# willwng/madrona_rl_envs_playground

Hardware: AMD Instinct MI355X
Metric: env-steps/sec (whole node), Overcooked 32768 worlds, random policy (higher is better)
Workload: dtype u8; 1 GPU; Overcooked cramped_room, 32768 worlds per GPU, horizon 400, uniform random actions (pre-sampled pool of 64, resident in HBM); worlds_per_gpu=32768, obs_gather=False

## Files before the change

### madrona_rl_envs_playground_amd/csrc/capi.hip

```cpp
#include "common.hpp"
#include "episode_scan.hpp"

#include <algorithm>
#include <cstring>
#include <exception>
#include <map>
#include <mutex>
#include <string>

namespace mrl {

static thread_local char g_error[512] = "";

static const char *const kDebugKeys[] = {
    "overcooked.wpw",
    "overcooked.whole_max",
    "overcooked.lds_max",
    "overcooked.share_max_players",
    "overcooked.share_private",
    "overcooked.no_share",
    "overcooked.lds_pad",
    "overcooked.no_fixed",
    "overcooked.no_direct",
    "overcooked.whole_store",
    "overcooked.store_policy",
    "overcooked.wide_rollout",
    "overcooked.groups",
    "overcooked.shared_consts",
    "overcooked.variant",
    "hanabi.variant",
    "hanabi.pairing",
    "hanabi.no_persistent",
    "cartpole.no_persistent",
    "cartpole.persistent_max",
    "cartpole.variant",
    "fused_step",
    "fused_heal_test",
    "inject_scan_timeout",
    "ablate",
    "stamps",
};
static std::mutex g_debug_mutex;
static std::map<std::string, int64_t> g_debug;

int64_t debug_get(const char *key, int64_t fallback)
{
    std::lock_guard<std::mutex> lock(g_debug_mutex);
    auto it = g_debug.find(key);
    return it == g_debug.end() ? fallback : it->second;
}

void set_error(const char *fmt, ...)
{
    va_list ap;
    va_start(ap, fmt);
    vsnprintf(g_error, sizeof(g_error), fmt, ap);
    va_end(ap);
}

void bind_device(int gpu_id)
{
    int count = 0;
// ... 484 lines not shown
```

### madrona_rl_envs_playground_amd/csrc/overcooked.hip

```cpp
#include "common.hpp"
#include "random_policy.hpp"
#include "world_reset.hpp"

#include <algorithm>
#include <cstdlib>
#include <cstring>

namespace {

constexpr int kWave = 64;
#ifndef MRL_OVERCOOKED_WPB
#define MRL_OVERCOOKED_WPB 4
#endif
constexpr int kWavesPerBlock = MRL_OVERCOOKED_WPB;
constexpr int kBlock = kWave * kWavesPerBlock;
constexpr int kRowsPerPass = 128;

enum : uint32_t { A_NORTH = 0, A_SOUTH = 1, A_EAST = 2, A_WEST = 3, A_STAY = 4, A_INTERACT = 5 };
enum : uint32_t { T_AIR = 0, T_POT, T_COUNTER, T_ONION_SRC, T_TOMATO_SRC, T_DISH_SRC, T_SERVING };
enum : uint32_t { O_NONE = 0, O_TOMATO, O_ONION, O_DISH, O_SOUP };
constexpr uint32_t kItemNone = 0xFF000000u;
constexpr uint32_t kMaxIngredients = 3;

constexpr uint32_t kConstTerrain = 0;
// ... 23 lines not shown
#endif
    uint32_t whole;
    uint32_t share;
    uint32_t team;
    uint32_t steady;
    uint32_t tail_even;
    uint32_t private_consts;
    uint32_t starts_w;
    uint32_t off_terr;
    uint32_t store_policy;
    uint32_t patch;
    uint32_t unaligned;
    const uint16_t *terr_off;
    uint32_t terr_entries;
    uint32_t direct;
    const uint32_t *hold_tab;
    uint32_t hold_entries;
    uint32_t off_pl, off_x, off_sum, off_cur, off_flags, off_list, off_tail, off_tile;
    uint32_t lds_wave_stride;
    int64_t horizon;
    const uint32_t *consts;
    uint32_t *cell_obj;
    uint2 *players;
    int32_t *timestep;
    const int32_t *actions;
    const long long *actions64;
    int32_t *action_mirror;
    int32_t *reward;
    int32_t *done;
    uint8_t *obs;
    uint64_t ring_stride;
    uint32_t ring_slots, ring_first;
    uint32_t pair_exchange;
};

__device__ __forceinline__ void wave_lds_sync()
{
    __builtin_amdgcn_wave_barrier();
    asm volatile("" ::: "memory");
}

__device__ __forceinline__ uint32_t lds_addr(const void *p)
{
    return (uint32_t)reinterpret_cast<uintptr_t>(p);
}

__device__ __forceinline__ void lds_store_tail_a4(uint8_t *ptr, const uint4 &t)
{
    asm volatile("ds_write_b32 %0, %1\n\t"
                 "ds_write_b32 %0, %2 offset:4\n\t"
                 "ds_write_b32 %0, %3 offset:8\n\t"
                 "ds_write_b32 %0, %4 offset:12"
                 :
                 : "v"(lds_addr(ptr)), "v"(t.x), "v"(t.y), "v"(t.z), "v"(t.w)
                 : "memory");
}

__device__ __forceinline__ void lds_store_tail_a2(uint8_t *ptr, const uint4 &t)
{
    const uint32_t m1 = __builtin_amdgcn_alignbit(t.y, t.x, 16);
    const uint32_t m2 = __builtin_amdgcn_alignbit(t.z, t.y, 16);
    const uint32_t m3 = __builtin_amdgcn_alignbit(t.w, t.z, 16);
    asm volatile("ds_write_b16 %0, %1\n\t"
                 "ds_write_b32 %0, %2 offset:2\n\t"
                 "ds_write_b32 %0, %3 offset:6\n\t"
                 "ds_write_b32 %0, %4 offset:10\n\t"
// ... 135 lines not shown
    const int32_t tick = (int8_t)(o >> 24);
    const uint32_t hname = h & 0xFF;
    const bool is_soup = oname == O_SOUP, in_pot = terr == T_POT;
    const bool idle = is_soup & in_pot & (tick < 0);
    const bool hot = is_soup & in_pot & (tick >= 0);
    const bool plated = is_soup & !in_pot;
    const bool hsoup = hname == O_SOUP;
    const uint32_t idle_on = idle ? on : 0u, idle_tom = idle ? tom : 0u;
    const uint32_t soup_on = hsoup ? (h >> 8) & 0xFF : ((hot | plated) ? on : 0u);
    const uint32_t soup_tom = hsoup ? (h >> 16) & 0xFF : ((hot | plated) ? tom : 0u);
    const uint32_t remaining = (hot & !hsoup) ? (uint32_t)(need - tick) & 0xFF : 0u;
    const uint32_t ready = (hsoup | plated | (hot & (tick >= need))) ? 1u : 0u;
    const uint32_t dish = ((oname == O_DISH) | (hname == O_DISH)) ? 1u : 0u;
    const uint32_t onion = ((oname == O_ONION) | (hname == O_ONION)) ? 1u : 0u;
    const uint32_t tomato = ((oname == O_TOMATO) | (hname == O_TOMATO)) ? 1u : 0u;
    const uint32_t tbit = terr == T_AIR ? 0u : 1u;
    const uint32_t tsh = ((terr - 1u) & 3u) * 8u;
    uint4 t;
    t.x = (terr >= 1 && terr <= 4) ? (tbit << tsh) : 0u;
    t.y = ((terr >= 5) ? (tbit << tsh) : 0u) | (idle_on << 16) | (idle_tom << 24);
    t.z = soup_on | (soup_tom << 8) | (remaining << 16) | (ready << 24);
    t.w = dish | (onion << 8) | (tomato << 16) | ((urgent ? 1u : 0u) << 24);
    return t;
}

__device__ __forceinline__ uint32_t swap_pair(uint32_t v)
{
    return (uint32_t)__builtin_amdgcn_mov_dpp((int)v, 0xB1, 0xF, 0xF, true);
}

template <int kP>
__device__ __forceinline__ void transition_lanes(const StepParams &p, const uint8_t *s_terrain, uint32_t *obj_w, uint32_t *s_x,
                                                 uint32_t *s_sum, uint32_t *s_blk, uint32_t P, uint32_t lane, bool active, uint32_t wl,
                                                 uint32_t q, uint32_t a, uint32_t &posori, uint32_t &held, int32_t &reward_world)
{
    const uint32_t pos = posori & 0xFFu, ori = (posori >> 8) & 0xFFu;
    const uint32_t tgt = pos + (uint32_t)step_of(ori, p.deltas);
    const uint32_t terr = s_terrain[tgt];
    const uint32_t ahead = s_terrain[pos + (uint32_t)step_of(a, p.deltas)];
    const bool inter = active && a == A_INTERACT;
    const bool touches = inter && (terr == T_COUNTER || terr == T_POT);
    const uint32_t key = touches ? tgt : 0xFFFFu;
    const uint32_t base = wl * P;
    uint32_t rank = 0;
    if constexpr (kP == 2) {
        const uint32_t other = swap_pair(key);
        rank = (q == 1u && touches && other == tgt) ? 1u : 0u;
    } else {
        s_x[lane] = key;
        wave_lds_sync();
        for (uint32_t q2 = 0; q2 + 1 < P; q2++) rank += (q2 < q && touches && s_x[base + q2] == key) ? 1u : 0u;
        wave_lds_sync();
    }
    int32_t mine = 0;
    const int32_t value = (int32_t)lookup16(p.values_w, recipe_of(held));
    uint32_t *cell = obj_w + (touches ? tgt : 0u);
    constexpr uint32_t kRounds = kP == 2 ? 2u : 4u;
#pragma clang loop unroll(disable)
    for (uint32_t r = 0; r < kRounds; r++) {
        const bool todo = inter && rank == r;
        if (r > 0 && __ballot(todo) == 0ull) break;
        if (todo) {
            uint32_t there = touches ? *cell : kItemNone;
            const int32_t need = (int32_t)lookup16(p.times_w, recipe_of(there));
            held = interact(p, need, value, terr, held, there, mine);
            if (touches) *cell = there;
        }
        wave_lds_sync();
    }
    uint32_t prop = pos, pori = ori;
    {
        const bool moves = a != A_INTERACT;
        const uint32_t np = pos + (uint32_t)step_of(a, p.deltas);
        pori = (moves && a != A_STAY) ? a : ori;
        prop = (moves && ahead == T_AIR) ? np : pos;
    }
    bool blocked;
    if constexpr (kP == 2) {
        reward_world = mine + (int32_t)swap_pair((uint32_t)mine);
        const uint32_t o = swap_pair(pos | (prop << 8));
        const uint32_t opos = o & 0xFFu, oprop = o >> 8;
        blocked = (prop == oprop) | ((prop == opos) & (pos == oprop));
    } else {
        s_x[lane] = pos | (prop << 8);
        if (active && q == 0) {
            s_sum[wl] = 0u;
            s_blk[wl] = 0u;
        }
        wave_lds_sync();
        if (mine != 0) atomicAdd(&s_sum[wl], (uint32_t)mine);
        bool hit = false;
        for (uint32_t q2 = 0; q2 < P; q2++) {
            const uint32_t v = s_x[base + q2];
            hit |= (q2 != q) & ((prop == (v >> 8)) | ((prop == (v & 0xFFu)) & (pos == (v >> 8))));
        }
        if (hit && active) s_blk[wl] = 1u;
        wave_lds_sync();
        reward_world = active ? (int32_t)s_sum[wl] : 0;
        blocked = active && s_blk[wl] != 0u;
        wave_lds_sync();
    }
    posori = (blocked ? pos : prop) | (pori << 8);
}

__device__ __forceinline__ void tick_pots_world(const StepParams &p, const uint8_t *s_pots, uint32_t *obj, bool valid)
{
    if (valid) {
        for (uint32_t k = 0; k < p.num_pots; k++) {
            const uint32_t c = k < 4 ? (p.pots_w >> (8 * k)) & 0xFFu : (uint32_t)s_pots[k];
            const uint32_t o = obj[c];
            const int32_t tick = (int8_t)(o >> 24);
            if ((o & 0xFF) == O_SOUP && tick >= 0 && tick < (int32_t)lookup16(p.times_w, recipe_of(o)))
                obj[c] = (o & 0x00FFFFFFu) | ((uint32_t)(uint8_t)(tick + 1) << 24);
        }
    }
}
__device__ __forceinline__ void tick_pots(const StepParams &p, const uint8_t *s_pots, uint32_t *s_obj, uint32_t nw, uint32_t lane)
{
    tick_pots_world(p, s_pots, s_obj + lane * p.C, lane < nw);
}
template <bool kPlain = false>
__device__ __forceinline__ void stream_store_rsrc(__amdgpu_buffer_rsrc_t rsrc, uint32_t byte_offset, const uint4 &v)
{
    u32x4 r;
    r.x = v.x;
    r.y = v.y;
    r.z = v.z;
    r.w = v.w;
#ifndef MRL_WHOLE_STORE_AUX
#define MRL_WHOLE_STORE_AUX 16
#endif
    __builtin_amdgcn_raw_buffer_store_b128(r, rsrc, (int)byte_offset, 0, kPlain ? 0 : MRL_WHOLE_STORE_AUX);
}

template <bool kPlain = false>
__device__ __forceinline__ void observe_whole(const StepParams &p, const uint8_t *s_terrain, const uint32_t *s_obj,
                                              const uint32_t *s_pl, const uint8_t *s_cur, const uint8_t *s_flags,
                                              uint8_t *s_tile, uint32_t P, uint32_t w0, uint32_t nw, uint32_t lane,
                                              bool prezeroed = false)
{
    const uint32_t C = p.C, F = p.F, shift = 5 * P, ncells = nw * C;
#ifdef MRL_DIAG
    if (p.ablate & 8u) return;
#endif
    uint8_t *gobs = p.obs + (size_t)w0 * p.block_bytes;
    const uint32_t nbytes = min(nw, w0 < p.num_worlds ? p.num_worlds - w0 : 0u) * p.block_bytes;
    const uint32_t mis = (uint32_t)(reinterpret_cast<uintptr_t>(gobs) & 15u);
    uint8_t *tile = s_tile + mis;
    if (!prezeroed) {
        const uint32_t nchunks = (mis + nbytes + 15u) >> 4;
        for (uint32_t k = lane; k < nchunks; k += kWave) reinterpret_cast<uint4 *>(s_tile)[k] = make_uint4(0, 0, 0, 0);
    }
    wave_lds_sync();
    const uint32_t plane = __umul24(C, F);
    for (uint32_t i = lane; i < ncells; i += kWave) {
        const uint32_t l = __umulhi(i, p.inv_c), c = i - __umul24(l, C);
        const uint32_t terr = s_terrain[c];
        const uint32_t o = s_obj[i];
        const uint32_t who = s_cur[i];
        const uint32_t urgent = s_flags[l];
        const bool occupied = who != 0xFF;
        const uint32_t pidx = (__umul24(l, P) + (occupied ? who : 0u)) * 2;
        const uint32_t w_ori = (s_pl[pidx] >> 8) & 0xFF;
        const uint32_t h = occupied ? s_pl[pidx + 1] : kItemNone;
        const uint4 t = cell_tail(p, terr, o, h, urgent);
// ... 49 lines not shown
        for (int k = 0; k < kBatch; k++) {
            if (i0 + (uint32_t)k * kWave >= ncells) break;
            const uint32_t i = i0 + (uint32_t)k * kWave + lane;
            const bool dyn = i < ncells && (((o[k] & 0xFFu) != O_NONE) | (who[k] != 0xFFu));
            const unsigned long long m = __ballot(dyn);
            const uint32_t before = __builtin_amdgcn_mbcnt_hi((uint32_t)(m >> 32), __builtin_amdgcn_mbcnt_lo((uint32_t)m, 0u));
            if (dyn) s_list[ndyn + before] = (uint16_t)i;
            ndyn += (uint32_t)__popcll(m);
        }
    }
    wave_lds_sync();
    return ndyn;
}

constexpr int kHoldPerLane = 4;
struct HoldTab {
    uint32_t e[kHoldPerLane];
};
__device__ __forceinline__ void hold_request(const StepParams &p, uint32_t lane, HoldTab &h)
{
    const __amdgpu_buffer_rsrc_t tab = __builtin_amdgcn_make_buffer_rsrc(const_cast<uint32_t *>(p.hold_tab), 0, (int)(p.hold_entries * 4u), 0x00020000);
#pragma unroll
    for (int k = 0; k < kHoldPerLane; k++) {
        if ((uint32_t)k * kWave >= p.hold_entries) {
            h.e[k] = 0;
            continue;
        }
        h.e[k] = (uint32_t)__builtin_amdgcn_raw_buffer_load_b32(tab, (int)((lane + (uint32_t)k * kWave) * 4u), 0, 0);
    }
}
template <int kP, bool kUndo>
__device__ __forceinline__ void patch_direct(const StepParams &p, uint32_t *s_obj, const uint8_t *s_flags, const HoldTab &hold,
                                             uint8_t *tile, uint32_t P, uint32_t nw, bool active, uint32_t wl, uint32_t q, uint32_t posori,
                                             uint32_t held)
{
    const uint32_t C = p.C, F = p.F, shift = 5 * P, ncells = nw * C;
    const uint32_t plane = __umul24(C, F);
    const uint32_t ori = (posori >> 8) & 0xFFu;
#pragma unroll
    for (int k = 0; k < kHoldPerLane; k++) {
        if (k > 0 && (uint32_t)k * kWave >= p.hold_entries) break;
        const uint32_t e = hold.e[k];
        const uint32_t i = (e >> 16) & 0x3FFFu;
        const bool holder = ((e >> 30) & 1u) != 0u && i < ncells;
        uint32_t o = s_obj[holder ? i : 0u];
        if (!kUndo && holder && (e >> 31)) {
            const int32_t tick = (int8_t)(o >> 24);
            if ((o & 0xFFu) == O_SOUP && tick >= 0 && tick < (int32_t)lookup16(p.times_w, recipe_of(o))) {
                o = (o & 0x00FFFFFFu) | ((uint32_t)(uint8_t)(tick + 1) << 24);
                s_obj[i] = o;
            }
        }
        const bool player = k == 0 && active;
        if (player || (holder && (o & 0xFFu) != O_NONE)) {
            const uint32_t l = player ? wl : __umulhi(i, p.inv_c);
            const uint32_t terr = player ? (uint32_t)T_AIR : ((e >> 31) ? (uint32_t)T_POT : (uint32_t)T_COUNTER);
            const uint4 t = cell_tail(p, terr, (player || kUndo) ? (uint32_t)kItemNone : o, (player && !kUndo) ? held : (uint32_t)kItemNone, s_flags[l]);
            uint8_t *row0 = tile + (player ? __umul24(l, p.block_bytes) + __umul24(posori & 0xFFu, F) : (e & 0xFFFFu));
            auto viewer_row = [&](uint32_t v, uint8_t *row) {
                lds_store_tail_even(row + shift, t);
                if (player) {
                    const uint32_t rel = q == v ? 0u : (q < v ? q + 1u : q);
                    row[rel] = kUndo ? 0 : 1;
                    row[P + 4 * rel + ori] = kUndo ? 0 : 1;
                }
            };
            if constexpr (kP == 2) {
                viewer_row(0, row0);
                viewer_row(1, row0 + plane);
            } else {
                for (uint32_t v = 0; v < P; v++) viewer_row(v, row0 + __umul24(v, plane));
            }
        }
    }
}

template <int kP, bool kRestore, bool kPlain = false>
__device__ __forceinline__ void observe_patch(const StepParams &p, const uint8_t *s_terrain, uint32_t *s_obj,
                                              const uint32_t *s_pl, const uint8_t *s_cur, const uint8_t *s_flags, uint8_t *s_prev,
                                              const uint16_t *s_list, uint32_t ndyn, uint8_t *tile, uint32_t P, uint32_t w0, uint32_t l0,
                                              uint32_t nl, uint32_t lane, const HoldTab &hold, bool active, uint32_t wl, uint32_t q,
                                              uint32_t posori, uint32_t held)
{
    const uint32_t C = p.C, F = p.F, shift = 5 * P;
#ifdef MRL_DIAG
    if (p.ablate & 8u) return;
#endif
    const uint32_t plane = __umul24(C, F);
    if (p.direct) patch_direct<kP, false>(p, s_obj, s_flags, hold, tile, P, nl, active, wl, q, posori, held);
    for (uint32_t j = lane; j < (p.direct ? 0u : ndyn); j += kWave) {
        const uint32_t i = s_list[j];
        const uint32_t l = __umulhi(i, p.inv_c), c = i - __umul24(l, C);
        const uint32_t terr = s_terrain[c];
        const uint32_t o = s_obj[i];
        const uint32_t who = s_cur[i];
        const uint32_t urgent = s_flags[l];
        const bool occupied = who != 0xFF;
        const uint32_t pidx = (__umul24(l, P) + (occupied ? who : 0u)) * 2;
        const uint32_t w_ori = (s_pl[pidx] >> 8) & 0xFF;
        const uint32_t h = occupied ? s_pl[pidx + 1] : kItemNone;
        const uint4 t = cell_tail(p, terr, o, h, urgent);
        uint8_t *row0 = tile + __umul24(l, p.block_bytes) + __umul24(c, F);
        auto viewer_row = [&](uint32_t v, uint8_t *row) {
            lds_store_tail_even(row + shift, t);
            if (occupied) {
                const uint32_t rel = who == v ? 0u : (who < v ? who + 1u : who);
                row[rel] = 1;
                row[P + 4 * rel + w_ori] = 1;
            }
        };
        if constexpr (kP == 2) {
            viewer_row(0, row0);
            viewer_row(1, row0 + plane);
        } else {
            for (uint32_t v = 0; v < P; v++) viewer_row(v, row0 + __umul24(v, plane));
        }
    }
    {
        const uint32_t mine = lane < nl ? s_flags[l0 + lane] : 0u;
        const uint32_t had = (kRestore && lane < nl) ? s_prev[l0 + lane] : 0u;
        if (__builtin_expect(__ballot(mine != had) != 0ull, 0)) {
            const uint32_t nrows = (l0 + nl) * p.rows;
            for (uint32_t r = l0 * p.rows + lane; r < nrows; r += kWave) {
                const uint32_t l = __umulhi(r, p.inv_rows);
                const uint32_t f = s_flags[l];
                if (f != (kRestore ? (uint32_t)s_prev[l] : 0u)) tile[__umul24(r, F) + F - 1u] = (uint8_t)f;
            }
            wave_lds_sync();
            if (kRestore && lane < nl) s_prev[l0 + lane] = (uint8_t)mine;
        }
    }
    wave_lds_sync();
#ifdef MRL_DIAG
    if (p.ablate & 2u) return;
#endif
    uint8_t *gobs = p.obs + (size_t)(w0 + l0) * p.block_bytes;
    const uint32_t nbytes = min(nl, w0 + l0 < p.num_worlds ? p.num_worlds - (w0 + l0) : 0u) * p.block_bytes;
    const uint8_t *from = tile + __umul24(l0, p.block_bytes);
    const uint32_t head = p.unaligned ? min((16u - ((uint32_t)reinterpret_cast<uintptr_t>(gobs) & 15u)) & 15u, nbytes) : 0u;
    if (lane < head) gobs[lane] = from[lane];
    const uint32_t body = (nbytes - head) >> 4;
    const uint4 *src = reinterpret_cast<const uint4 *>(from + head);
    const __amdgpu_buffer_rsrc_t out = __builtin_amdgcn_make_buffer_rsrc(gobs + head, 0, (int)(body << 4), 0x00020000);
#ifndef MRL_NO_LINE_ROUNDS
    const uint32_t lshift = kRestore ? 0u : (uint32_t)(reinterpret_cast<uintptr_t>(gobs + head) >> 4) & 7u;
#else
    const uint32_t lshift = 0u;
#endif
    int32_t b0 = -(int32_t)lshift;
    for (; b0 + 3 * kWave < (int32_t)body; b0 += 4 * kWave) {
        const int32_t ka = b0 + (int32_t)lane, kb = ka + kWave, kc = ka + 2 * kWave, kd = ka + 3 * kWave;
        const uint4 va = src[ka], vb = src[kb], vc = src[kc], vd = src[kd];
        stream_store_rsrc<kPlain>(out, (uint32_t)ka << 4, va);
        stream_store_rsrc<kPlain>(out, (uint32_t)kb << 4, vb);
        stream_store_rsrc<kPlain>(out, (uint32_t)kc << 4, vc);
        stream_store_rsrc<kPlain>(out, (uint32_t)kd << 4, vd);
    }
    for (; b0 < (int32_t)body; b0 += kWave) {
        const int32_t k = b0 + (int32_t)lane;
        stream_store_rsrc<kPlain>(out, (uint32_t)k << 4, src[k]);
    }
    const uint32_t done_bytes = head + (body << 4);
    if (lane < nbytes - done_bytes) gobs[done_bytes + lane] = from[done_bytes + lane];
    if constexpr (kRestore) {
        wave_lds_sync();
        if (p.direct) patch_direct<kP, true>(p, s_obj, s_flags, hold, tile, P, nl, active, wl, q, posori, held);
        for (uint32_t j = lane; j < (p.direct ? 0u : ndyn); j += kWave) {
            const uint32_t i = s_list[j];
            const uint32_t l = __umulhi(i, p.inv_c), c = i - __umul24(l, C);
            const uint32_t who = s_cur[i];
            const bool occupied = who != 0xFF;
            const uint32_t w_ori = (s_pl[(__umul24(l, P) + (occupied ? who : 0u)) * 2] >> 8) & 0xFF;
            const uint4 t = cell_tail(p, s_terrain[c], kItemNone, kItemNone, s_flags[l]);
            uint8_t *row0 = tile + __umul24(l, p.block_bytes) + __umul24(c, F);
            auto viewer_row = [&](uint32_t v, uint8_t *row) {
                lds_store_tail_even(row + shift, t);
                if (occupied) {
                    const uint32_t rel = who == v ? 0u : (who < v ? who + 1u : who);
                    row[rel] = 0;
                    row[P + 4 * rel + w_ori] = 0;
                }
            };
// ... 173 lines not shown
        if (p.patch) terrain_request(p, lane, tpos);
        if (!p.direct)
            for (uint32_t i = lane; i < (p.wpw * C + 3u) >> 2; i += kWave) reinterpret_cast<uint32_t *>(s_cur)[i] = 0xFFFFFFFFu;
        if (p.patch)
            tile_zero_addtid(s_tile, nw * p.block_bytes + patch_mis);
        else if (p.whole)
            tile_zero(p, lane, s_tile, nw);
        if (p.direct) hold_request(p, lane, hold);
        STAMP(6);
#pragma unroll
        for (int k = 0; k < kBatch; k++) {
            const uint32_t i = lane + k * kWave;
            if (i < ncells) s_obj[i] = cell_reg[k];
        }
        for (uint32_t i = lane + kBatch * kWave; i < ncells; i += kWave) s_obj[i] = g_obj[i];
        posori = pl_reg.x & 0xFFFFu;
        held = pl_reg.y;
        act = (active && a_raw <= A_INTERACT) ? a_raw : (uint32_t)A_STAY;
        if (p.actions64 && active && (!p.share || wib == 0)) p.action_mirror[a_at] = (int32_t)a_raw;
        if (!active) {
            posori = 0;
            held = kItemNone;
        }
    } else {
        if (p.patch) terrain_request(p, lane, tpos);
        if (!p.direct)
            for (uint32_t i = lane; i < (p.wpw * C + 3u) >> 2; i += kWave) reinterpret_cast<uint32_t *>(s_cur)[i] = 0xFFFFFFFFu;
        if (p.patch)
            tile_zero_addtid(s_tile, nw * p.block_bytes + patch_mis);
        else if (p.whole)
            tile_zero(p, lane, s_tile, nw);
        if (p.direct) hold_request(p, lane, hold);
    }
    if (p.patch) terrain_deliver(p, tpos, s_tile + patch_mis, nw);
    if (private_consts) {
        if (lane * 4u < p.C) reinterpret_cast<uint32_t *>(const_cast<uint8_t *>(s_terrain))[lane] = const_word[0];
        STAMP(7);
        wave_lds_sync();
    } else {
#pragma unroll
        for (int j = 0; j < kConstWordsPerThread; j++)
            if (tid + j * kBlock < kConstBytes / 4) reinterpret_cast<uint32_t *>(smem)[tid + j * kBlock] = const_word[j];
        STAMP(7);
        __syncthreads();
    }
    if (nw == 0) return;
    if (ABLATED(32)) return;
    STAMP(1);

    int32_t reward_world = 0, t = 0;
    bool reset_now = kInit;
    if (!kInit) {
        if (!ABLATED(4)) {
            transition_lanes<kP>(p, s_terrain, s_obj + wl * C, s_x, s_sum, s_blk, P, lane, active, wl, q, act, posori, held, reward_world);
            if (!p.direct) tick_pots(p, s_pots, s_obj, nw, lane);
        }
        t = t_loaded + 1;
        reset_now = (int64_t)t >= p.horizon;
    }
    if (__builtin_expect(__ballot(active && reset_now) != 0ull, 0)) {
        if (reset_now) {
            t = 0;
            posori = (private_consts ? (p.starts_w >> (8u * (q & 3u))) & 0xFFu : (uint32_t)s_start[active ? q : 0u]) | (A_NORTH << 8);
            held = kItemNone;
        }
        if (active && q == 0) s_sum[wl] = reset_now ? 1u : 0u;
        wave_lds_sync();
        for (uint32_t i = lane; i < ncells; i += kWave)
            if (s_sum[__umulhi(i, p.inv_c)] != 0u) s_obj[i] = kItemNone;
        wave_lds_sync();
    }
    STAMP(2);
    if (active) {
        if (!p.direct) {
            reinterpret_cast<uint2 *>(s_pl)[lane] = make_uint2(posori, held);
            s_cur[wl * C + (posori & 0xFFu)] = (uint8_t)q;
        }
        if (q == 0) s_flags[wl] = (p.horizon - (int64_t)t < 40) ? 1 : 0;
    }
    wave_lds_sync();

    auto store_state = [&]() {
        if (p.share && wib != 0) return;
        uint32_t *g_obj = p.cell_obj + (size_t)w0 * C;
#ifdef MRL_STATE_SC1
        for (uint32_t i = lane; i < ncells; i += kWave) asm volatile("global_store_dword %0, %1, off sc1" : : "v"(g_obj + i), "v"(s_obj[i]) : "memory");
        if (active) {
            const uint32_t world = w0 + wl;
            asm volatile("global_store_dwordx2 %0, %1, off sc1" : : "v"(p.players + (size_t)w0 * P + lane), "v"(make_uint2(posori, held)) : "memory");
            asm volatile("global_store_dword %0, %1, off sc1" : : "v"(p.reward + (size_t)q * N + world), "v"(reward_world) : "memory");
            if (q == 0) {
                asm volatile("global_store_dword %0, %1, off sc1" : : "v"(p.timestep + world), "v"(t) : "memory");
                asm volatile("global_store_dword %0, %1, off sc1" : : "v"(p.done + world), "v"(kInit ? 0 : (int32_t)reset_now) : "memory");
            }
        }
#else
        for (uint32_t i = lane; i < ncells; i += kWave) g_obj[i] = s_obj[i];
        if (active) {
            const uint32_t world = w0 + wl;
            p.players[(size_t)w0 * P + lane] = make_uint2(posori, held);
            p.reward[(size_t)q * N + world] = reward_world;
            if (q == 0) {
                p.timestep[world] = t;
                p.done[world] = kInit ? 0 : (int32_t)reset_now;
            }
        }
#endif
    };

    STAMP(3);
    const uint32_t F = p.F, shift = 5 * P;
    if (p.whole) {
        if (p.patch) {
            const uint32_t ndyn = p.direct ? 0u : find_dynamic(p, s_obj, s_cur, s_list, 0, nw, lane);
            STAMP(4);
            observe_patch<kP, false, kPlain>(p, s_terrain, s_obj, s_pl, s_cur, s_flags, nullptr, s_list, ndyn, s_tile + patch_mis, P, w0, 0, nw, lane, hold, active,
                                     wl, q, posori, held);
            STAMP(5);
        } else
            observe_whole<kPlain>(p, s_terrain, s_obj, s_pl, s_cur, s_flags, s_tile, P, w0, nw, lane, true);
        store_state();
        STAMP(15);
        STAMP_REALTIME(14);
        return;
    }
    for (uint32_t i = lane; i < ncells; i += kWave) {
        const uint32_t l = __umulhi(i, p.inv_c), c = i - __umul24(l, C);
        const uint32_t terr = s_terrain[c];
        const uint32_t o = s_obj[i];
        const uint32_t who = s_cur[i];
        const uint32_t urgent = s_flags[l];
        const uint32_t h = who != 0xFF ? s_pl[(__umul24(l, P) + who) * 2 + 1] : kItemNone;
        const uint4 t = cell_tail(p, terr, o, h, urgent);
        s_tail[i] = t;
    }
    wave_lds_sync();

    STAMP(4);
    constexpr uint32_t kRowsPerLane = kRowsPerPass / kWave;
    const uint32_t rows = p.rows;
    const uint32_t pass_rows = p.wpp ? p.wpp * rows : (uint32_t)kRowsPerPass;
    uint32_t k_wl[kRowsPerLane], k_viewer[kRowsPerLane], k_c[kRowsPerLane];
#pragma unroll
    for (uint32_t j = 0; j < kRowsPerLane; j++) {
        const uint32_t tr = lane * kRowsPerLane + j;
        const uint32_t wl = __umulhi(tr, p.inv_rows), r = tr - __umul24(wl, rows);
        k_wl[j] = wl;
        k_viewer[j] = __umulhi(r, p.inv_c);
        k_c[j] = r - __umul24(k_viewer[j], C);
    }
// ... 761 lines not shown
    bool generic = false;
    using StepKernel = void (*)(const StepParams);
    using RolloutKernel = void (*)(const StepParams, uint32_t, uint64_t, uint32_t, int32_t *, const int32_t *);
    StepKernel generic_step = nullptr;
    RolloutKernel generic_rollout = nullptr;
    using FixedKernel = void (*)(MRL_HOT_ARGS, const StepParams);
    FixedKernel fixed_kernel = nullptr;
    FixedKernel fixed_kernel_i64 = nullptr;
    FixedKernel groups_kernel = nullptr;
    FixedKernel groups_kernel_i64 = nullptr;
    uint32_t groups_grid = 0;
    const char *groups_name = nullptr;
    void (*fixed_rollout)(const StepParams, uint32_t, uint64_t, uint32_t, int32_t *, const int32_t *) = nullptr;
    void (*wide_rollout)(const StepParams, uint32_t, uint64_t, uint32_t, int32_t *, const int32_t *) = nullptr;
    StepParams wide_params{};
    uint32_t wide_grid = 0, wide_lds = 0;
    const char *fixed_name = nullptr;
    int32_t *action = nullptr, *active = nullptr, *mask = nullptr;
    int32_t *world_id = nullptr, *agent_id = nullptr, *loc_world_id = nullptr, *loc_id = nullptr;
    uint8_t *own_obs = nullptr;

    uint64_t observation_bytes() const override { return (uint64_t)num_worlds * params.block_bytes; }
    uint64_t set_observation_output(void *out) override
    {
        set_observation_ring(out, 0, 1);
        return observation_bytes();
    }
    uint8_t *ring_base = nullptr;
    uint64_t ring_stride = 0;
    uint32_t ring_slots = 1;
    uint64_t ring_pos = 0;
    bool staged = false;
    uint8_t *staging = nullptr, *pending_dest = nullptr;
    void set_observation_ring(void *base, uint64_t stride_bytes, uint32_t slots) override
    {
        ring_base = base ? static_cast<uint8_t *>(base) : own_obs;
        ring_stride = base ? stride_bytes : 0;
        ring_slots = base && slots > 1 ? slots : 1;
        ring_pos = 0;
        staged = base && ((reinterpret_cast<uintptr_t>(base) & 15u) != 0 || (ring_slots > 1 && (ring_stride & 15u) != 0));
        if (staged && !staging) staging = arena.alloc<uint8_t>(observation_bytes(), false);
        for (StepParams *q : {&params, &wide_params}) {
            q->obs = staged ? staging : ring_base;
            q->ring_stride = staged ? 0 : ring_stride;
            q->ring_slots = staged ? 1 : ring_slots;
            q->ring_first = 0;
        }
    }
    void deliver(uint8_t *dest, hipStream_t stream)
    {
        if (staged && dest) MRL_HIP(hipMemcpyAsync(dest, staging, observation_bytes(), hipMemcpyDeviceToDevice, stream));
    }

    mrl::FreshWorldOwner fresh;
    void reset_worlds(const uint8_t *mask, hipStream_t stream) override
    {
        if (staged)
            throw std::runtime_error("mrl_reset_worlds: the observation output is a staged slot (off a 16-byte boundary); a reset writes "
                                     "observations in place only -- use an aligned slot or the simulator's own tensor");
        const uint64_t slot = ring_pos ? (ring_pos - 1) % ring_slots : 0;
        fresh.launch(mask, num_worlds, ring_base + (size_t)slot * ring_stride, stream);
    }
    uint8_t *take_slots(uint32_t steps, uint32_t *first)
    {
        const uint32_t at = (uint32_t)(ring_pos % ring_slots);
        ring_pos += steps;
        if (first) *first = at;
        return ring_base + (size_t)at * ring_stride;
    }

    StepParams generic_step_params(const int32_t *actions)
    {
        StepParams a = params;
        a.actions = actions ? actions : action;
        pending_dest = take_slots(1, nullptr);
        a.obs = staged ? staging : pending_dest;
        a.ring_slots = 1;
        a.per_xcd = grid >> 3;
        a.pair_exchange = (a.P == 2 && !generic) ? 1u : 0u;
        return a;
    }

    void launch(bool init, const int32_t *actions, hipStream_t stream)
    {
        StepParams a = params;
        a.actions = actions ? actions : action;
        uint8_t *const dest = init ? nullptr : take_slots(1, nullptr);
        if (!init) a.obs = staged ? staging : dest;
        a.ring_slots = 1;
        a.per_xcd = ((!init && groups_kernel) ? groups_grid : grid) >> 3;
        const void *hot_actions = a.actions64 ? static_cast<const void *>(a.actions64) : static_cast<const void *>(a.actions);
        if (a.team && init)
            hipLaunchKernelGGL((mrl_overcooked_step_team<true>), dim3(grid), dim3(kBlock), lds_bytes, stream, a);
        else if (a.team)
            hipLaunchKernelGGL((mrl_overcooked_step_team<false>), dim3(grid), dim3(kBlock), lds_bytes, stream, a);
        else if (init)
            hipLaunchKernelGGL((mrl_overcooked_step<true, 0>), dim3(grid), dim3(kBlock), lds_bytes, stream, a);
        else if (groups_kernel)
            hipLaunchKernelGGL(a.actions64 ? groups_kernel_i64 : groups_kernel, dim3(groups_grid), dim3(kBlock), lds_bytes, stream, a.cell_obj,
                               a.players, a.timestep, hot_actions, a.consts, a.terr_off, a.num_worlds, a.per_xcd, a);
        else if (fixed_kernel)
            hipLaunchKernelGGL(a.actions64 ? fixed_kernel_i64 : fixed_kernel, dim3(grid), dim3(kBlock), lds_bytes, stream, a.cell_obj, a.players,
                               a.timestep, hot_actions, a.consts, a.terr_off, a.num_worlds, a.per_xcd, a);
        else
            hipLaunchKernelGGL(generic_step, dim3(grid), dim3(kBlock), lds_bytes, stream, a);
        MRL_HIP(hipGetLastError());
        deliver(dest, stream);
    }

    void phase1(const int32_t *actions, hipStream_t stream) override { launch(false, actions, stream); }
    bool step_i64(const long long *actions, hipStream_t stream) override
    {
        const long long *keep = params.actions64;
        params.actions64 = actions;
        params.action_mirror = action;
        launch(false, nullptr, stream);
        params.actions64 = keep;
        return true;
    }
    void phase2(const uint32_t *, hipStream_t) override {}

    void rollout_random(uint32_t num_steps, uint64_t seed, uint32_t first_step, hipStream_t stream) override
    {
        if (num_steps == 0) return;
        if (params.whole && !staged) {
            take_slots(num_steps, &params.ring_first);
            wide_params.ring_first = params.ring_first;
            if (wide_rollout)
                hipLaunchKernelGGL(wide_rollout, dim3(wide_grid), dim3(kWavesPerBlock * kWave), wide_lds, stream, wide_params, num_steps,
                                   seed, first_step, action, (const int32_t *)nullptr);
            else if (fixed_rollout)
                hipLaunchKernelGGL(fixed_rollout, dim3(grid), dim3(kWavesPerBlock * kWave), lds_bytes, stream, params, num_steps, seed,
                                   first_step, action, (const int32_t *)nullptr);
            else
                hipLaunchKernelGGL(generic_rollout, dim3(grid), dim3(kWavesPerBlock * kWave), lds_bytes, stream, params, num_steps, seed,
                                   first_step, action, (const int32_t *)nullptr);
            MRL_HIP(hipGetLastError());
            return;
        }
        const size_t count = (size_t)params.P * num_worlds;
        for (uint32_t k = 0; k < num_steps; k++) {
            hipLaunchKernelGGL(mrl_overcooked_draw_actions, dim3((unsigned)((count + 255) / 256)), dim3(256), 0, stream,
                               action, params.P, num_worlds, seed, first_step + k);
            launch(false, nullptr, stream);
        }
    }

    void step_sequence(const int32_t *actions, uint32_t num_steps, hipStream_t stream) override
    {
        if (num_steps == 0) return;
        if (params.whole && !staged) {
            take_slots(num_steps, &params.ring_first);
            wide_params.ring_first = params.ring_first;
            if (wide_rollout)
                hipLaunchKernelGGL(wide_rollout, dim3(wide_grid), dim3(kWavesPerBlock * kWave), wide_lds, stream, wide_params, num_steps,
                                   0ull, 0u, action, actions);
            else if (fixed_rollout)
                hipLaunchKernelGGL(fixed_rollout, dim3(grid), dim3(kWavesPerBlock * kWave), lds_bytes, stream, params, num_steps, 0ull, 0u,
                                   action, actions);
            else
                hipLaunchKernelGGL(generic_rollout, dim3(grid), dim3(kWavesPerBlock * kWave), lds_bytes, stream, params, num_steps, 0ull, 0u,
                                   action, actions);
            MRL_HIP(hipGetLastError());
            return;
        }
        mrl_sim::step_sequence(actions, num_steps, stream);
    }

    void ensure_ids()
    {
        if (world_id) return;
        const uint32_t P = params.P, N = num_worlds, rows = params.rows;
        world_id = arena.alloc<int32_t>((size_t)P * N, false);
        agent_id = arena.alloc<int32_t>((size_t)P * N, false);
        loc_world_id = arena.alloc<int32_t>((size_t)rows * N, false);
        loc_id = arena.alloc<int32_t>((size_t)rows * N, false);
        const size_t a = (size_t)P * N, b = (size_t)rows * N;
        hipLaunchKernelGGL(fill_ids, dim3((unsigned)((a + 255) / 256)), dim3(256), 0, 0, world_id, agent_id, P, N);
        hipLaunchKernelGGL(fill_ids, dim3((unsigned)((b + 255) / 256)), dim3(256), 0, 0, loc_world_id, loc_id, rows, N);
        MRL_HIP(hipGetLastError());
        MRL_HIP(hipDeviceSynchronize());
    }

    bool tensor(int slot, mrl_tensor_desc *out) override
    {
// ... 230 lines not shown
            if (tab.empty()) tab.resize(1, 0u);
            return tab;
        };
        {
            bool starts_walkable = true;
            for (int64_t q = 0; q < P; q++) starts_walkable = starts_walkable && consts[kConstTerrain + consts[kConstStart + q]] == T_AIR;
            a.direct = (a.patch && starts_walkable && hold_table(a.wpw).size() <= (size_t)kHoldPerLane * kWave &&
                        !mrl::debug_get("overcooked.no_direct", 0))
                           ? 1u
                           : 0u;
        }
        const auto plain_for = [&](uint32_t group_worlds, bool multi_step) {
            const int64_t knob = mrl::debug_get("overcooked.whole_store", 0);
            const uint64_t slab = (uint64_t)N * a.block_bytes;
            const bool whole_lines = ((uint64_t)group_worlds * a.block_bytes) % 64u == 0;
            return knob ? knob == 2 : (!whole_lines && (multi_step || slab > (256ull << 20)));
        };
        const bool plain = plain_for(wpw, false), plain_multi = plain_for(wpw, true);
        {
            const bool pairs = a.P == 2 && !sim->generic;
            sim->generic_step = pairs ? (plain ? &mrl_overcooked_step<false, 2, true> : &mrl_overcooked_step<false, 2, false>)
                                      : (plain ? &mrl_overcooked_step<false, 0, true> : &mrl_overcooked_step<false, 0, false>);
            sim->generic_rollout = pairs ? (plain_multi ? &mrl_overcooked_rollout<2, true> : &mrl_overcooked_rollout<2, false>)
                                         : (plain_multi ? &mrl_overcooked_rollout<0, true> : &mrl_overcooked_rollout<0, false>);
        }
        if (sim->lds_bytes > 65536) {
            MRL_HIP(hipFuncSetAttribute(reinterpret_cast<const void *>(sim->generic_step), hipFuncAttributeMaxDynamicSharedMemorySize, (int)sim->lds_bytes));
            MRL_HIP(hipFuncSetAttribute(reinterpret_cast<const void *>(&mrl_overcooked_step<true, 0>), hipFuncAttributeMaxDynamicSharedMemorySize,
                                        (int)sim->lds_bytes));
            MRL_HIP(hipFuncSetAttribute(reinterpret_cast<const void *>(sim->generic_rollout), hipFuncAttributeMaxDynamicSharedMemorySize,
                                        (int)sim->lds_bytes));
        }
        a.share = (wpw == 1 && !a.whole && a.wpp == 0 && N < 8192 && P <= (uint32_t)mrl::debug_get("overcooked.share_max_players", 64) && !mrl::debug_get("overcooked.no_share", 0)) ? 1u : 0u;
        if (a.share && !mrl::debug_get("overcooked.share_private", 0)) {
            auto up16 = [](uint32_t v) { return (v + 15u) & ~15u; };
            a.team = 1;
            a.off_pl = up16(a.C * 4);
            a.off_x = a.off_pl + up16(a.P * 8);
            a.off_sum = a.off_x + 128u * 4u;
            a.off_cur = a.off_sum + 16u;
            a.off_flags = a.off_cur + up16(a.C);
            a.off_tail = a.off_flags + 64u;
            a.off_tile = a.off_tail + a.C * 16u;
            a.lds_wave_stride = tile_bytes;
            sim->lds_bytes = kConstBytes + a.off_tile + kWavesPerBlock * tile_bytes + (uint32_t)mrl::debug_get("overcooked.lds_pad", 0);
            if (sim->lds_bytes > 65536) {
                MRL_HIP(hipFuncSetAttribute(reinterpret_cast<const void *>(&mrl_overcooked_step_team<false>), hipFuncAttributeMaxDynamicSharedMemorySize,
                                            (int)sim->lds_bytes));
                MRL_HIP(hipFuncSetAttribute(reinterpret_cast<const void *>(&mrl_overcooked_step_team<true>), hipFuncAttributeMaxDynamicSharedMemorySize,
                                            (int)sim->lds_bytes));
            }
        }
        {
            auto matches = [&](uint32_t C_, uint32_t wpw_, uint32_t width_, uint32_t pots_, uint32_t hold_) {
                const FixedLayout f = fixed_layout(C_, wpw_);
                return a.P == 2 && !sim->generic && a.C == C_ && a.W == width_ && a.num_pots == pots_ && a.wpw == wpw_ && a.whole &&
                       a.patch && !a.unaligned && a.direct && holders.size() == hold_ && !a.share && a.private_consts && a.off_pl == f.off_pl && a.off_sum == f.off_sum &&
                       a.off_cur == f.off_cur && a.off_flags == f.off_flags && a.off_terr == f.off_terr && a.off_list == f.off_list &&
                       a.off_tile == f.off_tile && a.lds_wave_stride == f.stride && !mrl::debug_get("overcooked.no_fixed", 0);
            };
#define MRL_FIXED(C_, WPW_, WIDTH_, POTS_, HOLD_)                                                                    \
    if (!sim->fixed_kernel && matches(C_, WPW_, WIDTH_, POTS_, HOLD_)) {                                            \
        sim->fixed_kernel = plain ? &mrl_overcooked_step_fixed<C_, WPW_, WIDTH_, POTS_, HOLD_, false, true>         \
                                  : &mrl_overcooked_step_fixed<C_, WPW_, WIDTH_, POTS_, HOLD_, false, false>;       \
        sim->fixed_kernel_i64 = plain ? &mrl_overcooked_step_fixed<C_, WPW_, WIDTH_, POTS_, HOLD_, true, true>      \
                                      : &mrl_overcooked_step_fixed<C_, WPW_, WIDTH_, POTS_, HOLD_, true, false>;    \
// ... 168 lines not shown
```

Baseline: 4.073 billion env-steps/s.

## Write only dirty observation cache lines when the output buffer is unchanged

Adds a dirty-line bitmask per block that records which 128-byte lines of the observation tile change during a step (player moves, held item changes, cell writes, pot ticks, urgency flips, resets). When the host can show the destination buffer still holds the previous step's observations (not captured, not staged, single ring slot, same pointer), the kernel stores only the dirty lines instead of streaming the whole observation. This cuts HBM write traffic at the cost of LDS atomics, host-side capture checks, and correctness depending on the buffer tracking.

```diff
diff --git a/madrona_rl_envs_playground_amd/csrc/capi.hip b/madrona_rl_envs_playground_amd/csrc/capi.hip
--- a/madrona_rl_envs_playground_amd/csrc/capi.hip
+++ b/madrona_rl_envs_playground_amd/csrc/capi.hip
@@ -28,6 +28,7 @@
     "overcooked.groups",
     "overcooked.shared_consts",
     "overcooked.variant",
+    "overcooked.full_obs",
     "hanabi.variant",
     "hanabi.pairing",
     "hanabi.no_persistent",
diff --git a/madrona_rl_envs_playground_amd/csrc/overcooked.hip b/madrona_rl_envs_playground_amd/csrc/overcooked.hip
--- a/madrona_rl_envs_playground_amd/csrc/overcooked.hip
+++ b/madrona_rl_envs_playground_amd/csrc/overcooked.hip
@@ -79,6 +79,7 @@
     uint64_t ring_stride;
     uint32_t ring_slots, ring_first;
     uint32_t pair_exchange;
+    uint32_t obs_delta;
 };
 
 __device__ __forceinline__ void wave_lds_sync()
@@ -280,7 +281,8 @@
 template <int kP>
 __device__ __forceinline__ void transition_lanes(const StepParams &p, const uint8_t *s_terrain, uint32_t *obj_w, uint32_t *s_x,
                                                  uint32_t *s_sum, uint32_t *s_blk, uint32_t P, uint32_t lane, bool active, uint32_t wl,
-                                                 uint32_t q, uint32_t a, uint32_t &posori, uint32_t &held, int32_t &reward_world)
+                                                 uint32_t q, uint32_t a, uint32_t &posori, uint32_t &held, int32_t &reward_world,
+                                                 uint32_t *written_cell = nullptr)
 {
     const uint32_t pos = posori & 0xFFu, ori = (posori >> 8) & 0xFFu;
     const uint32_t tgt = pos + (uint32_t)step_of(ori, p.deltas);
@@ -311,8 +313,10 @@
         if (todo) {
             uint32_t there = touches ? *cell : kItemNone;
             const int32_t need = (int32_t)lookup16(p.times_w, recipe_of(there));
+            const uint32_t found = there;
             held = interact(p, need, value, terr, held, there, mine);
             if (touches) *cell = there;
+            if (written_cell && touches && there != found) *written_cell = tgt;
         }
         wave_lds_sync();
     }
@@ -379,6 +383,48 @@
 #define MRL_WHOLE_STORE_AUX 16
 #endif
     __builtin_amdgcn_raw_buffer_store_b128(r, rsrc, (int)byte_offset, 0, kPlain ? 0 : MRL_WHOLE_STORE_AUX);
+}
+
+constexpr uint32_t kDirtyWords = 3;
+struct DirtyLines {
+    uint32_t *words = nullptr;
+    uint32_t origin = 0;
+    bool on = false;
+};
+__device__ __forceinline__ void dirty_mark(const DirtyLines &d, uint32_t first, uint32_t count)
+{
+    const uint32_t a = (first + d.origin) >> 7, b = (first + count - 1u + d.origin) >> 7;
+#pragma unroll
+    for (uint32_t j = 0; j < kDirtyWords; j++) {
+        const uint32_t lo = max(a, 32u * j), hi = min(b, 32u * j + 31u);
+        if (lo <= hi) atomicOr(&d.words[j], ((2u << (hi - lo)) - 1u) << (lo - 32u * j));
+    }
+}
+__device__ __forceinline__ void dirty_mark_cell(const StepParams &p, const DirtyLines &d, uint32_t P, uint32_t l, uint32_t c)
+{
+    const uint32_t plane = __umul24(p.C, p.F);
+    uint32_t row = __umul24(l, p.block_bytes) + __umul24(c, p.F);
+    for (uint32_t v = 0; v < P; v++, row += plane) dirty_mark(d, row, p.F);
+}
+__device__ __forceinline__ void dirty_mark_lane(const StepParams &p, const DirtyLines &d, uint32_t P, uint32_t wl, uint32_t q,
+                                                uint32_t posori_was, uint32_t held_was, uint32_t posori, uint32_t held,
+                                                uint32_t written_cell, bool whole_world)
+{
+    if (posori != posori_was || held != held_was) {
+        dirty_mark_cell(p, d, P, wl, posori_was & 0xFFu);
+        if (((posori ^ posori_was) & 0xFFu) != 0u) dirty_mark_cell(p, d, P, wl, posori & 0xFFu);
+    }
+    if (written_cell != 0xFFFFFFFFu) dirty_mark_cell(p, d, P, wl, written_cell);
+    if (q == 0 && whole_world) dirty_mark(d, __umul24(wl, p.block_bytes), p.block_bytes);
+}
+template <bool kRestore>
+__device__ __forceinline__ uint32_t line_shift(const uint8_t *first_chunk)
+{
+#ifndef MRL_NO_LINE_ROUNDS
+    return kRestore ? 0u : (uint32_t)(reinterpret_cast<uintptr_t>(first_chunk) >> 4) & 7u;
+#else
+    return 0u;
+#endif
 }
 
 template <bool kPlain = false>
@@ -494,7 +540,7 @@
 template <int kP, bool kUndo>
 __device__ __forceinline__ void patch_direct(const StepParams &p, uint32_t *s_obj, const uint8_t *s_flags, const HoldTab &hold,
                                              uint8_t *tile, uint32_t P, uint32_t nw, bool active, uint32_t wl, uint32_t q, uint32_t posori,
-                                             uint32_t held)
+                                             uint32_t held, const DirtyLines &dirty = DirtyLines{})
 {
     const uint32_t C = p.C, F = p.F, shift = 5 * P, ncells = nw * C;
     const uint32_t plane = __umul24(C, F);
@@ -511,6 +557,8 @@
             if ((o & 0xFFu) == O_SOUP && tick >= 0 && tick < (int32_t)lookup16(p.times_w, recipe_of(o))) {
                 o = (o & 0x00FFFFFFu) | ((uint32_t)(uint8_t)(tick + 1) << 24);
                 s_obj[i] = o;
+                if (dirty.on)
+                    for (uint32_t v = 0; v < P; v++) dirty_mark(dirty, (e & 0xFFFFu) + __umul24(v, plane), F);
             }
         }
         const bool player = k == 0 && active;
@@ -542,14 +590,14 @@
                                               const uint32_t *s_pl, const uint8_t *s_cur, const uint8_t *s_flags, uint8_t *s_prev,
                                               const uint16_t *s_list, uint32_t ndyn, uint8_t *tile, uint32_t P, uint32_t w0, uint32_t l0,
                                               uint32_t nl, uint32_t lane, const HoldTab &hold, bool active, uint32_t wl, uint32_t q,
-                                              uint32_t posori, uint32_t held)
+                                              uint32_t posori, uint32_t held, const DirtyLines &dirty = DirtyLines{})
 {
     const uint32_t C = p.C, F = p.F, shift = 5 * P;
 #ifdef MRL_DIAG
     if (p.ablate & 8u) return;
 #endif
     const uint32_t plane = __umul24(C, F);
-    if (p.direct) patch_direct<kP, false>(p, s_obj, s_flags, hold, tile, P, nl, active, wl, q, posori, held);
+    if (p.direct) patch_direct<kP, false>(p, s_obj, s_flags, hold, tile, P, nl, active, wl, q, posori, held, dirty);
     for (uint32_t j = lane; j < (p.direct ? 0u : ndyn); j += kWave) {
         const uint32_t i = s_list[j];
         const uint32_t l = __umulhi(i, p.inv_c), c = i - __umul24(l, C);
@@ -604,12 +652,34 @@
     const uint32_t body = (nbytes - head) >> 4;
     const uint4 *src = reinterpret_cast<const uint4 *>(from + head);
     const __amdgpu_buffer_rsrc_t out = __builtin_amdgcn_make_buffer_rsrc(gobs + head, 0, (int)(body << 4), 0x00020000);
-#ifndef MRL_NO_LINE_ROUNDS
-    const uint32_t lshift = kRestore ? 0u : (uint32_t)(reinterpret_cast<uintptr_t>(gobs + head) >> 4) & 7u;
-#else
-    const uint32_t lshift = 0u;
-#endif
+    const uint32_t lshift = line_shift<kRestore>(gobs + head);
     int32_t b0 = -(int32_t)lshift;
+    if (dirty.on) {
+        uint32_t mask[kDirtyWords];
+#pragma unroll
+        for (uint32_t j = 0; j < kDirtyWords; j++) mask[j] = (uint32_t)__builtin_amdgcn_readfirstlane((int)dirty.words[j]);
+        constexpr uint32_t kDropped = 0xFFFFFFF0u;
+#pragma unroll
+        for (uint32_t j = 0; j < kDirtyWords; j++, b0 += 4 * kWave) {
+            if (b0 >= (int32_t)body) break;
+            const uint32_t word = mask[j];
+            if (word == 0u) continue;
+            const uint32_t mine = word >> (lane >> 3);
+            uint4 v[4];
+#pragma unroll
+            for (int r = 0; r < 4; r++) {
+                v[r] = make_uint4(0, 0, 0, 0);
+                if (((word >> (8 * r)) & 0xFFu) != 0u && ((mine >> (8 * r)) & 1u) != 0u) v[r] = src[b0 + r * kWave + (int32_t)lane];
+            }
+#pragma unroll
+            for (int r = 0; r < 4; r++) {
+                if (((word >> (8 * r)) & 0xFFu) == 0u) continue;
+                const int32_t k = b0 + r * kWave + (int32_t)lane;
+                stream_store_rsrc<kPlain>(out, ((mine >> (8 * r)) & 1u) != 0u ? (uint32_t)k << 4 : kDropped, v[r]);
+            }
+        }
+        b0 = (int32_t)body;
+    }
     for (; b0 + 3 * kWave < (int32_t)body; b0 += 4 * kWave) {
         const int32_t ka = b0 + (int32_t)lane, kb = ka + kWave, kc = ka + 2 * kWave, kd = ka + 3 * kWave;
         const uint4 va = src[ka], vb = src[kb], vc = src[kc], vd = src[kd];
@@ -849,6 +919,14 @@
             tile_zero(p, lane, s_tile, nw);
         if (p.direct) hold_request(p, lane, hold);
     }
+    const uint32_t posori_was = posori, held_was = held;
+    DirtyLines dirty{};
+    if (!kInit && p.obs_delta) {
+        dirty.words = reinterpret_cast<uint32_t *>(s_list);
+        dirty.origin = line_shift<false>(p.obs + (size_t)w0 * p.block_bytes) << 4;
+        dirty.on = true;
+        if (lane < kDirtyWords) dirty.words[lane] = 0u;
+    }
     if (p.patch) terrain_deliver(p, tpos, s_tile + patch_mis, nw);
     if (private_consts) {
         if (lane * 4u < p.C) reinterpret_cast<uint32_t *>(const_cast<uint8_t *>(s_terrain))[lane] = const_word[0];
@@ -867,9 +945,11 @@
 
     int32_t reward_world = 0, t = 0;
     bool reset_now = kInit;
+    uint32_t written_cell = 0xFFFFFFFFu;
     if (!kInit) {
         if (!ABLATED(4)) {
-            transition_lanes<kP>(p, s_terrain, s_obj + wl * C, s_x, s_sum, s_blk, P, lane, active, wl, q, act, posori, held, reward_world);
+            transition_lanes<kP>(p, s_terrain, s_obj + wl * C, s_x, s_sum, s_blk, P, lane, active, wl, q, act, posori, held, reward_world,
+                                 &written_cell);
             if (!p.direct) tick_pots(p, s_pots, s_obj, nw, lane);
         }
         t = t_loaded + 1;
@@ -887,6 +967,9 @@
             if (s_sum[__umulhi(i, p.inv_c)] != 0u) s_obj[i] = kItemNone;
         wave_lds_sync();
     }
+    if (dirty.on && active)
+        dirty_mark_lane(p, dirty, P, wl, q, posori_was, held_was, posori, held, written_cell,
+                        reset_now || (p.horizon - (int64_t)t_loaded < 40) != (p.horizon - (int64_t)t < 40));
     STAMP(2);
     if (active) {
         if (!p.direct) {
@@ -932,7 +1015,7 @@
             const uint32_t ndyn = p.direct ? 0u : find_dynamic(p, s_obj, s_cur, s_list, 0, nw, lane);
             STAMP(4);
             observe_patch<kP, false, kPlain>(p, s_terrain, s_obj, s_pl, s_cur, s_flags, nullptr, s_list, ndyn, s_tile + patch_mis, P, w0, 0, nw, lane, hold, active,
-                                     wl, q, posori, held);
+                                     wl, q, posori, held, dirty);
             STAMP(5);
         } else
             observe_whole<kPlain>(p, s_terrain, s_obj, s_pl, s_cur, s_flags, s_tile, P, w0, nw, lane, true);
@@ -1760,8 +1843,23 @@
     uint64_t ring_pos = 0;
     bool staged = false;
     uint8_t *staging = nullptr, *pending_dest = nullptr;
+    bool delta_ok = false;
+    bool graph_seen = false;
+    const uint8_t *obs_current = nullptr;
+    bool capturing(hipStream_t stream)
+    {
+        if (!stream) return graph_seen;
+        hipStreamCaptureStatus status = hipStreamCaptureStatusNone;
+        if (hipStreamIsCapturing(stream, &status) != hipSuccess) {
+            (void)hipGetLastError();
+            status = hipStreamCaptureStatusActive;
+        }
+        if (status != hipStreamCaptureStatusNone) graph_seen = true;
+        return graph_seen;
+    }
     void set_observation_ring(void *base, uint64_t stride_bytes, uint32_t slots) override
     {
+        obs_current = nullptr;
         ring_base = base ? static_cast<uint8_t *>(base) : own_obs;
         ring_stride = base ? stride_bytes : 0;
         ring_slots = base && slots > 1 ? slots : 1;
@@ -1787,7 +1885,9 @@
             throw std::runtime_error("mrl_reset_worlds: the observation output is a staged slot (off a 16-byte boundary); a reset writes "
                                      "observations in place only -- use an aligned slot or the simulator's own tensor");
         const uint64_t slot = ring_pos ? (ring_pos - 1) % ring_slots : 0;
-        fresh.launch(mask, num_worlds, ring_base + (size_t)slot * ring_stride, stream);
+        uint8_t *const dest = ring_base + (size_t)slot * ring_stride;
+        if (capturing(stream) || dest != obs_current) obs_current = nullptr;
+        fresh.launch(mask, num_worlds, dest, stream);
     }
     uint8_t *take_slots(uint32_t steps, uint32_t *first)
     {
@@ -1806,6 +1906,7 @@
         a.ring_slots = 1;
         a.per_xcd = grid >> 3;
         a.pair_exchange = (a.P == 2 && !generic) ? 1u : 0u;
+        obs_current = nullptr;
         return a;
     }
 
@@ -1816,6 +1917,9 @@
         uint8_t *const dest = init ? nullptr : take_slots(1, nullptr);
         if (!init) a.obs = staged ? staging : dest;
         a.ring_slots = 1;
+        const bool recorded = capturing(stream);
+        a.obs_delta = (!init && delta_ok && !groups_kernel && !recorded && !staged && ring_slots <= 1 && dest == obs_current) ? 1u : 0u;
+        obs_current = (recorded || staged) ? nullptr : (init ? own_obs : dest);
         a.per_xcd = ((!init && groups_kernel) ? groups_grid : grid) >> 3;
         const void *hot_actions = a.actions64 ? static_cast<const void *>(a.actions64) : static_cast<const void *>(a.actions);
         if (a.team && init)
@@ -1836,6 +1940,12 @@
         deliver(dest, stream);
     }
 
+    void multi_step_wrote(uint32_t num_steps, hipStream_t stream)
+    {
+        const uint64_t last = ((uint64_t)params.ring_first + num_steps - 1) % ring_slots;
+        obs_current = capturing(stream) ? nullptr : ring_base + (size_t)last * ring_stride;
+    }
+
     void phase1(const int32_t *actions, hipStream_t stream) override { launch(false, actions, stream); }
     bool step_i64(const long long *actions, hipStream_t stream) override
     {
@@ -1853,6 +1963,7 @@
         if (num_steps == 0) return;
         if (params.whole && !staged) {
             take_slots(num_steps, &params.ring_first);
+            multi_step_wrote(num_steps, stream);
             wide_params.ring_first = params.ring_first;
             if (wide_rollout)
                 hipLaunchKernelGGL(wide_rollout, dim3(wide_grid), dim3(kWavesPerBlock * kWave), wide_lds, stream, wide_params, num_steps,
@@ -1879,6 +1990,7 @@
         if (num_steps == 0) return;
         if (params.whole && !staged) {
             take_slots(num_steps, &params.ring_first);
+            multi_step_wrote(num_steps, stream);
             wide_params.ring_first = params.ring_first;
             if (wide_rollout)
                 hipLaunchKernelGGL(wide_rollout, dim3(wide_grid), dim3(kWavesPerBlock * kWave), wide_lds, stream, wide_params, num_steps,
@@ -2175,6 +2287,8 @@
                                         (int)sim->lds_bytes));
         }
         a.share = (wpw == 1 && !a.whole && a.wpp == 0 && N < 8192 && P <= (uint32_t)mrl::debug_get("overcooked.share_max_players", 64) && !mrl::debug_get("overcooked.no_share", 0)) ? 1u : 0u;
+        sim->delta_ok = a.whole && a.patch && a.direct && !a.unaligned && !a.share && (uint64_t)N * a.block_bytes >= (32ull << 20) &&
+                        ((uint64_t)wpw * a.block_bytes + 112u + 127u) / 128u <= 32u * kDirtyWords && !mrl::debug_get("overcooked.full_obs", 0);
         if (a.share && !mrl::debug_get("overcooked.share_private", 0)) {
             auto up16 = [](uint32_t v) { return (v + 15u) & ~15u; };
             a.team = 1;
```

Result: faster. 4.397 billion env-steps/s, median of 6 (+8.0%).
